# fahmyadan/SMARTS

Hardware: AMD Instinct MI355X
Metric: aggregate env-steps/s (all agents) (higher is better)
Workload: dtype f64; 1 GPU; scenarios/loop, 4096 batched envs x 32 Laner agents, waypoints(4x20, lookahead 32)+neighbours(10, r=50 m) obs, OGM 64x64 @ 50/64 m/px, dt=0.1, auto-reset (BASELINE.json configs[3]); total_envs=4096, envs_per_gpu=4096, vehicles_per_env=32, launch_form=large_one_lane

## Files before the change

### include/smx.h

```cpp
#ifndef SMX_H
#define SMX_H

#include <stdint.h>

#ifdef __cplusplus
extern "C" {
#endif

typedef struct smx_handle_s* smx_handle;

typedef enum smx_status {
  SMX_OK = 0,
  SMX_ERR_INVALID = -1,
  SMX_ERR_HIP = -2,
  SMX_ERR_STATE = -3,
  SMX_ERR_NOMEM = -4
} smx_status;

enum {
  SMX_ACTION_KEEP_LANE = 0,
  SMX_ACTION_SLOW_DOWN = 1,
  SMX_ACTION_CHANGE_LANE_LEFT = 2,
  SMX_ACTION_CHANGE_LANE_RIGHT = 3,
  SMX_ACTION_NONE = -1
// ... 424 lines not shown
                         int32_t max_points, double* out_dev, const smx_outputs* out, void* hip_stream);
int smx_sync(smx_handle h, void* hip_stream);
enum {
  SMX_PHASE_CONTROL = 0,
  SMX_PHASE_SCAN,
  SMX_PHASE_OGM,
  SMX_PHASE_SENSORS,
  SMX_PHASE_COMMIT,
  SMX_PHASE_RESET,
  SMX_PHASE_COUNT
};
int smx_set_timing(smx_handle h, int level);
int smx_read_phase_ms(smx_handle h, float* ms, int32_t max_steps, int32_t* n);
int smx_read_step_ms(smx_handle h, float* ms, int32_t max, int32_t* n);
int smx_last_step_ms(smx_handle h, float* ms);
const char* smx_last_error(smx_handle h);
uint64_t smx_struct_size(int which);
int smx_set_controller_gains(smx_handle h, double heading_gain, double lateral_gain);
enum { SMX_LAUNCH_AUTO = 0, SMX_LAUNCH_SMALL = 1, SMX_LAUNCH_LARGE = 2,
       SMX_LAUNCH_LARGE_ONE_LANE = 3, SMX_LAUNCH_LARGE_TEAMS = 4  };
int smx_set_launch_strategy(smx_handle h, int strategy);
enum { SMX_FORM_SMALL = 0, SMX_FORM_LARGE_TEAMS = 1, SMX_FORM_LARGE_ONE_LANE = 2 };
int smx_launch_form(smx_handle h);
const char* smx_version(void);
void smx_destroy(smx_handle h);

#ifdef __cplusplus
}
#endif
#endif
```

### smarts_amd/_native.py

```python
from __future__ import annotations

import ctypes as C
import os
from typing import Optional

from .build import LIB_PATH

ACTION_KEEP_LANE, ACTION_SLOW_DOWN, ACTION_CHANGE_LANE_LEFT, ACTION_CHANGE_LANE_RIGHT = 0, 1, 2, 3
ACTION_NONE = -1
DONE_COLLISION, DONE_OFF_ROAD, DONE_OFF_ROUTE = 1, 2, 4
DONE_ON_SHOULDER, DONE_WRONG_WAY, DONE_NOT_MOVING = 8, 16, 32
(EV_COLLISIONS, EV_OFF_ROAD, EV_OFF_ROUTE, EV_ON_SHOULDER, EV_WRONG_WAY, EV_NOT_MOVING, EV_REACHED_GOAL,
 EV_REACHED_MAX_EPISODE_STEPS, EV_AGENTS_ALIVE_DONE, EV_COUNT) = range(10)
EVENT_NAMES = ["collisions", "off_road", "off_route", "on_shoulder", "wrong_way", "not_moving", "reached_goal",
               "reached_max_episode_steps", "agents_alive_done"]
EV = {name.upper(): i for i, name in enumerate(EVENT_NAMES)}
ACTION_SPACES = {"Lane": 0, "Continuous": 1, "ActuatorDynamic": 2, "LaneWithContinuousSpeed": 3, "Trajectory": 4,
                 "TargetPose": 5, "TrajectoryWithTime": 6, "MPC": 7, "Imitation": 8}
TRAJ_COLS = 11
SOCIAL_MODELS = {"constant": 0, "idm": 1}
PHASES = ["control", "scan", "ogm", "sensors", "commit", "reset"]
SENSOR_WAYPOINTS, SENSOR_NEIGHBORS, SENSOR_ACCELEROMETER, SENSOR_OGM, SENSOR_LIDAR, SENSOR_DAGM = 1, 2, 4, 8, 16, 32
SENSOR_ROAD_WAYPOINTS = 64
SENSOR_LANE_TTC = 128
# ... 144 lines not shown

def torch_dtype_code(t) -> int:
    import torch

    return {torch.float64: DT_F64, torch.float32: DT_F32, torch.int32: DT_I32, torch.int16: DT_I16, torch.int8: DT_I8,
            torch.uint8: DT_U8, torch.int64: DT_U64, torch.uint64: DT_U64}[t.dtype]


def bind_buffer(struct, names, name, tensor):
    k = names.index(name)
    setattr(struct, name, tensor.data_ptr() if tensor is not None else None)
    struct.count[k] = int(tensor.numel()) if tensor is not None else 0
    struct.dtype[k] = torch_dtype_code(tensor) if tensor is not None else DT_NONE


EXPORTS = [
    "smx_create", "smx_load_map", "smx_set_vias", "smx_set_missions", "smx_step_continuous", "smx_step_trajectory", "smx_read_phase_ms", "smx_set_lidar_rays", "smx_reset", "smx_step", "smx_sync", "smx_last_step_ms",
    "smx_set_timing", "smx_last_error", "smx_version", "smx_destroy", "smx_set_controller_gains", "smx_struct_size", "smx_read_step_ms",
    "smx_check_buffers", "smx_set_launch_strategy", "smx_launch_form", "smx_step_target_pose", "smx_step_trajectory_with_time",
    "smx_set_mission_goals", "smx_check_mission_goals", "smx_actions_to_world", "smx_set_rgb_output", "smx_check_rgb_output",
    "smx_bind_frame_stack", "smx_check_frame_stack", "smx_set_guard", "smx_check_guard",
    "smx_set_social_history", "smx_check_social_history", "smx_set_social_history_dims", "smx_check_social_history_dims",
    "smx_set_history_agents", "smx_check_history_agents", "smx_step_history_agents",
]
LAUNCH_FORMS = {0: "small", 1: "large_teams", 2: "large_one_lane"}
LAUNCH_STRATEGIES = {"auto": 0, "small": 1, "large": 2, "large_one_lane": 3, "large_teams": 4}
OGM_ENV_MIN_VEHICLES = 8192
LARGE_BATCH_VEHICLES = 16384

_lib: Optional[C.CDLL] = None


class NativeLibraryError(RuntimeError):
    pass


def load_library(path: Optional[str] = None) -> C.CDLL:
    global _lib
    if _lib is not None and path is None:
        return _lib
    path = path or os.environ.get("SMX_LIBRARY") or LIB_PATH
    if not os.path.exists(path):
        raise NativeLibraryError(
            f"{path} not found: build it with `python -m smarts_amd.build` (hipcc --offload-arch=gfx950); "
            "smarts_amd has no CPU fallback"
        )
# ... 68 lines not shown
                                             C.c_char_p, C.c_uint64]
    lib.smx_check_history_agents.restype = C.c_int
    lib.smx_step_history_agents.argtypes = [h, C.POINTER(SmxState), C.POINTER(SmxSpawns), C.POINTER(SmxOutputs), _p]
    lib.smx_step_history_agents.restype = C.c_int
    lib.smx_read_phase_ms.argtypes = [h, C.POINTER(C.c_float), _i32, C.POINTER(_i32)]
    lib.smx_read_phase_ms.restype = C.c_int
    lib.smx_set_timing.argtypes = [h, C.c_int]
    lib.smx_set_timing.restype = C.c_int
    lib.smx_set_controller_gains.argtypes = [h, _f64, _f64]
    lib.smx_set_controller_gains.restype = C.c_int
    lib.smx_last_error.argtypes = [h]
    lib.smx_last_error.restype = C.c_char_p
    lib.smx_version.argtypes = []
    lib.smx_version.restype = C.c_char_p
    lib.smx_destroy.argtypes = [h]
    lib.smx_destroy.restype = None
    lib.smx_check_buffers.argtypes = [C.POINTER(SmxConfig), C.c_int, C.POINTER(SmxState), C.POINTER(SmxSpawns),
                                      C.POINTER(SmxOutputs), C.c_char_p, C.c_uint64]
    lib.smx_check_buffers.restype = C.c_int
    lib.smx_set_launch_strategy.argtypes = [h, C.c_int]
    lib.smx_set_launch_strategy.restype = C.c_int
    lib.smx_launch_form.argtypes = [h]
    lib.smx_launch_form.restype = C.c_int
    lib.smx_struct_size.argtypes = [C.c_int]
    lib.smx_struct_size.restype = C.c_uint64
    for which, mirror in enumerate((SmxConfig, SmxMapTables, SmxState, SmxSpawns, SmxOutputs)):
        if lib.smx_struct_size(which) != C.sizeof(mirror):
            raise NativeLibraryError(
                f"ABI mismatch: {mirror.__name__} is {C.sizeof(mirror)} bytes here, "
                f"{lib.smx_struct_size(which)} in {path} (stale build?)"
            )
    _lib = lib
    return lib


class SmxError(RuntimeError):
    pass


def check(lib, handle, rc: int, what: str):
    if rc != 0:
        msg = lib.smx_last_error(handle)
        raise SmxError(f"{what} failed ({rc}): {msg.decode() if msg else ''}")
```

### smarts_amd/csrc/smx_kernels.hip

```cpp
#include <hip/hip_runtime.h>

#include <algorithm>
#include <cmath>
#include <cstdio>
#include <cstdlib>
#include <cstring>
#include <new>
#include <string>
#include <vector>

#include "smx_guard.h"
#include "smx_history.h"
#include "smx_host.h"
#include "smx_plan.h"
#include "smx_scan.h"
#include "smx_vehicle.h"

#define SMX_COLLISION_LEEWAY 0.05
#define SMX_POSE_SCAN_RADIUS 10.0
#define SMX_WPT_PRELOAD 8
#define SMX_SLOW_BLOCKS 512

struct KernelArgs {
  smx_config cfg;
// ... 21 lines not shown
  int debug_skip;
  int wp_blocks, obs_blocks, lidar_blocks;
  double dagm_reach;
  uint8_t* rgb;
  KnotLists knots;
  const KnotRow* knot_table;
  unsigned long long* knot_served;
  MissionsDev missions;
  const int32_t* alive_list;
  const int32_t* alive_count;
  int alive_segmented;
  int32_t* status;
  double* seeds_carry;
  double* facts_carry;
  int32_t* slow_list;
  int32_t* slow_count;
  uint8_t* seed_pending;
  uint8_t* guard;
  GuardBox guard_box;
  HistoryDev history;
  HistoryDimsDev dims;
  float* ha_action;
  uint8_t* ha_status;
};
enum {
  SMX_DEVICE_BAD_LANE_ACTION = 1,
  SMX_DEVICE_BAD_TRAJECTORY = 2,
  SMX_DEVICE_BAD_TARGET_POSE = 4
};

#define SF(field) a.st.f64[(size_t)(field) * total + gid]

#define SMX_SEG_STRIDE 32
__device__ __forceinline__ size_t seg_position(const size_t seg, const size_t off) {
  return ((off >> 6) << 9) | (seg << 6) | (off & 63);
}

__device__ __forceinline__ size_t launch_vehicle(const KernelArgs& a, size_t i, size_t total) {
  if (a.alive_list == nullptr) return i < total ? i : total;
  const int32_t entry = a.alive_list[i < total ? i : total - 1];
  if (a.alive_segmented) {
    const size_t off = ((i >> 9) << 6) | (i & 63);
    return (i < total && off < (size_t)a.alive_count[SMX_SEG_STRIDE * ((i >> 6) & 7)]) ? (size_t)entry : total;
  }
  return i < (size_t)*a.alive_count ? (size_t)entry : total;
}
// ... 2758 lines not shown
      SF(SMX_S_MCL_Y) = so[1];
      fl |= SMX_F_SOCIAL;
    }
  } else if (__builtin_expect(a.history.follow != nullptr, 0)) {
    fl = history_agent_respawn(a, gid, total, episode);
    if constexpr (GUARD) a.guard[gid] = 0;
  }
  a.st.flags[gid] = fl;
  if (a.knots.key != nullptr)
    for (int p = 0; p < SMX_WP_LANES; ++p) a.knots.key[gid * SMX_WP_LANES + p] = -1;
  a.st.facts_i32[(size_t)SMX_FI_TRIP_HAS_WP * total + gid] = 0;
  a.st.steps[gid] = 1;
}

struct __align__(16) SharedPose {
  double x, y, heading, speed;
  double lane_dist;
  int lane;
  int alive;
  short nl, nlidx;
  int pad;
};

__device__ __forceinline__ void zero_dense_rows(const KernelArgs& a, size_t gid, int t, int nth) {
  const smx_config& c = a.cfg;
  const smx_outputs& o = a.out;
  for (int k = t; k < 3; k += nth) o.ego_pos[gid * 3 + k] = 0.0;
  for (int k = t; k < SMX_EGO_F32_COUNT; k += nth) o.ego_f32[gid * SMX_EGO_F32_COUNT + k] = 0.0f;
  for (int k = t; k < 2; k += nth) o.ego_lane[gid * 2 + k] = -1;
  for (int k = t; k < SMX_EV_COUNT; k += nth) o.events[gid * SMX_EV_COUNT + k] = 0;
  if (t == 0) {
    if (o.collidees) o.collidees[gid] = 0ull;
    o.reward[gid] = 0.0;
    o.dist[gid] = 0.0;
  }
  if (c.sensors & SMX_SENSOR_WAYPOINTS) {
    const int per = c.wp_paths * c.wp_len;
    for (int k = t; k < per * 3; k += nth) o.wp_pos[gid * per * 3 + k] = 0.0;
    for (int k = t; k < per; k += nth) {
      const size_t q = gid * per + k;
      o.wp_heading[q] = 0.0f;
      o.wp_lane_width[q] = 0.0f;
      o.wp_speed_limit[q] = 0.0f;
      o.wp_lane_index[q] = 0;
      o.wp_lane_id[q] = -1;
    }
// ... 10 lines not shown
      o.nb_speed[q] = 0.0f;
      o.nb_lane_index[q] = 0;
      o.nb_lane_id[q] = -1;
      o.nb_slot[q] = -1;
    }
    if (t == 0) o.nb_count[gid] = 0;
  }
  if ((c.sensors & SMX_SENSOR_LANE_TTC) && t == 0) o.lane_ttc_flags[gid] = 0;
  if (c.via_max > 0 && o.via_near) {
    for (int k = t; k < c.via_max; k += nth) o.via_near[gid * (size_t)c.via_max + k] = -1;
    if (t == 0) {
      o.via_near_count[gid] = 0;
      o.via_hit[gid] = 0;
    }
  }
  auto zero_bytes = [&](uint8_t* base, size_t n) {
    uint8_t* p = base + gid * n;
    if (n % 16 == 0 && (reinterpret_cast<uintptr_t>(p) & 15) == 0) {
      for (size_t k = t; k < n / 16; k += nth) reinterpret_cast<int4*>(p)[k] = make_int4(0, 0, 0, 0);
    } else {
      for (size_t k = t; k < n; k += nth) p[k] = 0;
    }
  };
  if ((c.sensors & SMX_SENSOR_OGM) && o.ogm) zero_bytes(o.ogm, (size_t)c.ogm_width * c.ogm_height);
  if ((c.sensors & SMX_SENSOR_DAGM) && o.dagm) zero_bytes(o.dagm, (size_t)c.dagm_width * c.dagm_height);
  if ((c.sensors & SMX_SENSOR_LIDAR) && o.lidar_hit) {
    for (int k = t; k < c.lidar_rays; k += nth) o.lidar_hit[gid * (size_t)c.lidar_rays + k] = 0;
    for (int k = t; k < c.lidar_rays * 3; k += nth) o.lidar_point[gid * (size_t)c.lidar_rays * 3 + k] = 0.0;
  }
}

#define SMX_NB_STAGE 16
static_assert(SMX_BLOCK * SMX_NB_STAGE * 3 < 4096, "small_quotient's range");
struct ObsStage {
  float ego_f32[SMX_BLOCK][SMX_EGO_F32_COUNT];
  short ego_lane[SMX_BLOCK][2];
  unsigned char events[SMX_BLOCK][SMX_EV_COUNT + 1];
  signed char nb_list[SMX_BLOCK][SMX_NB_STAGE];
  unsigned char nb_kept[SMX_BLOCK];
  unsigned char mode[SMX_BLOCK];
};

__device__ inline bool drove_off_map(const MissionsDev& ms, const MapDev& m, int n_slots, int lane, double dist, double px,
                                     double py, double heading) {
  if (lane < 0) return false;
  const double offset = lane_offset_along(m, lane, px, py);
  const double width = m.lane_width[lane];
// ... 640 lines not shown
  const double res = c.ogm_resolution;
  const double ex0 = SF(SMX_S_X), ey0 = SF(SMX_S_Y), eh = wrap_heading(SF(SMX_S_HEADING));
  const double rx = cos(eh), ry = sin(eh);
  const double fx = -sin(eh), fy = cos(eh);
  __shared__ OgmMate mates[SMX_BLOCK];
  for (int base = 0; base < n_veh; base += SMX_BLOCK) {
    const int j = base + (int)threadIdx.x;
    bool in_view = false;
    if (j < n_veh) {
      const size_t og = (size_t)env * n_veh + j;
      if (a.st.flags[og] & SMX_F_ALIVE) in_view = ogm_mate_footprint(a, og, total, W, H, res, ex0, ey0, rx, ry, fx, fy, mates[threadIdx.x]);
    }
    unsigned long long todo = __ballot(in_view);
    __syncthreads();
    while (todo != 0ull) {
      const int idx = __ffsll((long long)todo) - 1;
      const OgmMate q = mates[idx];
      todo &= todo - 1ull;
      ogm_draw_mate<255>(a, (size_t)env * n_veh + base + idx, tile, q, W, H, res);
    }
    __syncthreads();
  }
  __syncthreads();
  int4* dst = reinterpret_cast<int4*>(a.out.ogm + gid * (size_t)bytes);
  for (int k = threadIdx.x; k < bytes / 16; k += SMX_BLOCK) dst[k] = reinterpret_cast<const int4*>(tile)[k];
}

struct OgmPose {
  double x, y, ch, sh;
  int alive, observes;
};
#ifndef SMX_SIDE_PRIO
#define SMX_SIDE_PRIO 0
#endif
#define SMX_WAVE_SYNC()                                   \
  do {                                                    \
    __builtin_amdgcn_fence(__ATOMIC_RELEASE, "wavefront"); \
    __builtin_amdgcn_wave_barrier();                      \
    __builtin_amdgcn_fence(__ATOMIC_ACQUIRE, "wavefront"); \
  } while (0)
__device__ __forceinline__ double readlane_f64(double v, int src) {
  const long long b = __double_as_longlong(v);
  const int lo = __builtin_amdgcn_readlane((int)(b & 0xffffffffll), src);
  const int hi = __builtin_amdgcn_readlane((int)(b >> 32), src);
  return __longlong_as_double(((long long)hi << 32) | (unsigned int)lo);
}

template <int OBS, bool SIZED>
// ... 22 lines not shown
    p.sh = sin(h);
    pose[threadIdx.x] = p;
  }
  if (wave == 0) {
    const bool obs_here = lane < n_veh && pose[lane].observes;
    const unsigned long long om = __ballot(obs_here);
    if (obs_here) observers[__popcll(om & ((1ull << lane) - 1ull))] = (unsigned char)lane;
    if (lane == 0) n_observers = __popcll(om);
  }
  __syncthreads();
  unsigned char* tile = tiles + (size_t)wave * OBS * bytes;
  const double res = c.ogm_resolution;
  const double inv_res = 1.0 / res;
  const int half = lane >> 5, in_half = lane & 31;
  const int mate = OBS == 2 ? in_half : lane;
  const int mate_clamped = min(mate, n_veh - 1);
  const VehBox mate_box = vehicle_box(a, (size_t)env * n_veh + mate_clamped, SIZED);
  const double hl = 0.5 * mate_box.length, hw = 0.5 * mate_box.width;
  const int lr = in_half >> 2, lc = in_half & 3;
  const double col_bias = 0.5 - 0.5 * W, row_bias = 0.5 * H - 0.5;
  const int n_obs = n_observers;
  const int per_round = SMX_OGM_WAVES * OBS;
  const int rounds = (n_obs + per_round - 1) / per_round;
#pragma nounroll
  for (int it = 0; it < rounds; ++it) {
    const int turn0 = (it * SMX_OGM_WAVES + wave) * OBS;
    const int n_live = min(OBS, n_obs - turn0);
    if (n_live <= 0) break;
    for (int k = lane; k < n_live * (bytes / 16); k += 64) reinterpret_cast<int4*>(tile)[k] = make_int4(0, 0, 0, 0);
    const int my_turn = turn0 + (OBS == 2 ? half : 0);
    const bool live = my_turn < n_obs;
    const int obs = (int)observers[live ? my_turn : turn0];
    const OgmPose e = pose[obs];
    const OgmPose v = pose[mate_clamped];
    const double rx = e.ch, ry = e.sh;
    const double fx = -e.sh, fy = e.ch;
    const double dx = v.x - e.x, dy = v.y - e.y;
    const double cx = dx * rx + dy * ry, cy = dx * fx + dy * fy;
    const double cm = v.ch, sm = v.sh;
    const double vfx = cm * ry - sm * rx, vfy = sm * ry + cm * rx, vrx = cm * rx + sm * ry, vry = sm * rx - cm * ry;
    const double ext_x = fabs(vfx) * hl + fabs(vrx) * hw, ext_y = fabs(vfy) * hl + fabs(vry) * hw;
    const double slack = 1e-6;
    const double c_lo = fmax((cx - ext_x) * inv_res + 0.5 * W - 0.5 - slack, -1.0), c_hi = fmin((cx + ext_x) * inv_res + 0.5 * W - 0.5 + slack, (double)W);
    const double r_lo = fmax(0.5 * H - 0.5 - (cy + ext_y) * inv_res - slack, -1.0), r_hi = fmin(0.5 * H - 0.5 - (cy - ext_y) * inv_res + slack, (double)H);
    const int c0 = max((int)ceil(c_lo), 0), c1 = min((int)floor(c_hi), W - 1);
    const int r0 = max((int)ceil(r_lo), 0), r1 = min((int)floor(r_hi), H - 1);
// ... 13 lines not shown
      const double qvfx = __shfl(vfx, src), qvfy = __shfl(vfy, src), qvrx = __shfl(vrx, src), qvry = __shfl(vry, src);
      const int qc0 = __shfl(c0, src), qr0 = __shfl(r0, src), qbw = __shfl(bw, src), qbh = __shfl(bh, src);
      double qhl = 0.5 * SMX_CHASSIS_LENGTH, qhw = 0.5 * SMX_CHASSIS_WIDTH;
      if constexpr (SIZED) qhl = __shfl(hl, src), qhw = __shfl(hw, src);
      unsigned char* dst_tile = tile + (OBS == 2 ? (src >> 5) * bytes : 0);
      const int bh_max = max(__builtin_amdgcn_readlane(bh, s0), __builtin_amdgcn_readlane(bh, s1));
      const int bw_max = max(__builtin_amdgcn_readlane(bw, s0), __builtin_amdgcn_readlane(bw, s1));
#pragma clang loop unroll(disable) vectorize(disable) interleave(disable)
      for (int rr = 0; rr < bh_max; rr += 8) {
#pragma clang loop unroll(disable) vectorize(disable) interleave(disable)
        for (int cc = 0; cc < bw_max; cc += 4) {
          const int dr = rr + lr, dc = cc + lc;
          const int r = qr0 + dr, col = qc0 + dc;
          const double py = (row_bias - (double)r) * res - qcy;
          const double px = ((double)col + col_bias) * res - qcx;
          if (drawing && dr < qbh && dc < qbw && fabs(px * qvfx + py * qvfy) <= qhl && fabs(px * qvrx + py * qvry) <= qhw)
            dst_tile[r * W + col] = 255;
        }
      }
    }
    SMX_WAVE_SYNC();
    for (int t = 0; t < n_live; ++t) {
      const int4* src_tile = reinterpret_cast<const int4*>(tile + (size_t)t * bytes);
      int4* dst = reinterpret_cast<int4*>(a.out.ogm + ((size_t)env * n_veh + (int)observers[turn0 + t]) * (size_t)bytes);
      for (int k = lane; k < bytes / 16; k += 64) dst[k] = src_tile[k];
    }
    SMX_WAVE_SYNC();
  }
  SMX_TSTAMP(span1);
  SMX_TSPAN(6, span0, span1);
}

template <int VALUE>
__device__ __forceinline__ void road_layer(const KernelArgs& a, unsigned char* tile, const int W, const int H, const double res,
                                           const double ex0, const double ey0, const double rx, const double ry, const double fx,
                                           const double fy) {
  const MapDev& m = a.map;
  const double vw = 0.5 * W * res, vh = 0.5 * H * res;
  const double reach = sqrt(vw * vw + vh * vh) + a.dagm_reach + 1e-6;
  int cx0 = (int)floor((ex0 - reach - m.sg_x0) / m.sg_cell), cx1 = (int)floor((ex0 + reach - m.sg_x0) / m.sg_cell);
  int cy0 = (int)floor((ey0 - reach - m.sg_y0) / m.sg_cell), cy1 = (int)floor((ey0 + reach - m.sg_y0) / m.sg_cell);
  cx0 = max(cx0, 0);
  cy0 = max(cy0, 0);
  cx1 = min(cx1, m.sg_nx - 1);
  cy1 = min(cy1, m.sg_ny - 1);
  const int wave = threadIdx.x >> 6, lane = threadIdx.x & 63, n_waves = SMX_BLOCK >> 6;
  for (int gy = cy0; gy <= cy1; ++gy) {
    if (cx0 > cx1) break;
// ... 1130 lines not shown
  void* goals_blob;
  std::vector<int32_t> host_route_last;
  MissionsDev missions;
  double heading_gain_pos = 0.04, lateral_gain_pos = 3.4;
  double nb_d2_max;
  int slow_blocks = SMX_SLOW_BLOCKS;
  bool list_ready;
  int seg_parity;
  smx_state list_state;
  int group_parity;
  bool map_junctions;
  double dagm_reach;
  uint8_t* guard_out;
  uint64_t guard_count;
  double guard_margin = SMX_GUARD_MARGIN_DEFAULT;
  GuardBox guard_box = {1.0, 1.0, 0.0, 0.0};
  uint8_t* rgb_out;
  uint64_t rgb_count;
  void* history_blob;
  HistoryDev history;
  float* ha_action;
  uint8_t* ha_status;
  int32_t history_max_id;
  void* dims_blob;
  HistoryDimsDev dims;
  struct StackBinding {
    int32_t source, layout;
    uint8_t* dst;
    uint64_t bytes;
    uint32_t row;
  };
  std::vector<StackBinding> stacks;
  int debug_skip;
  int launch_strategy = SMX_LAUNCH_AUTO;
  bool timing;
  std::vector<hipEvent_t> ev_pool;
  size_t ev_used;
  bool phase_timing;
  std::vector<hipEvent_t> ph_pool;
  size_t ph_used;
  std::string err;
};

static thread_local std::string g_create_err;

static void drop_social_dims(smx_handle h) {
// ... 71 lines not shown
  l.flat = total;
  l.seg = (total + 2 + SMX_SEG_STRIDE - 1) / SMX_SEG_STRIDE * SMX_SEG_STRIDE;
  l.group_count = l.seg + 2 * 8 * SMX_SEG_STRIDE;
  l.groups = l.group_count + 2 * SMX_SEG_STRIDE;
  l.size = l.groups + (size_t)c.num_envs;
  return l;
}

static_assert(SMX_HOST_BLOCK == SMX_BLOCK && SMX_HOST_WP_LANES == SMX_WP_LANES && SMX_HOST_MAX_KNOTS == SMX_MAX_KNOTS &&
                  SMX_HOST_SLOW_BLOCKS == SMX_SLOW_BLOCKS && SMX_HOST_STACK_BLOCK == SMX_STACK_BLOCK,
              "smx_host.h mirrors these");

extern "C" int smx_create(const smx_config* cfg, int device, smx_handle* out) {
  if (out) *out = nullptr;
  if (!cfg || !out) return refuse(g_create_err, "smx_create: null config or handle pointer");
  if (const char* why = config_error(*cfg)) return refuse(g_create_err, why);
  const hipError_t e = hipSetDevice(device);
  if (e != hipSuccess) return refuse(g_create_err, std::string("hipSetDevice: ") + hipGetErrorString(e), SMX_ERR_HIP);
  smx_handle h = new (std::nothrow) smx_handle_s();
  if (!h) return refuse(g_create_err, "out of memory", SMX_ERR_NOMEM);
  h->cfg = *cfg;
  h->device = device;
  h->nb_d2_max = radius_threshold(h->cfg.nb_radius);
#ifdef SMX_DEBUG_TIMING
  if (const char* dbg = getenv("SMX_DEBUG_SKIP")) h->debug_skip = atoi(dbg);
#endif
  *out = h;
  return SMX_OK;
}

extern "C" int smx_set_launch_strategy(smx_handle h, int strategy) {
  if (!h) return SMX_ERR_INVALID;
  if (strategy < SMX_LAUNCH_AUTO || strategy > SMX_LAUNCH_LARGE_TEAMS) return fail(h, SMX_ERR_INVALID, "unknown launch strategy");
  h->launch_strategy = strategy;
  return SMX_OK;
}

static PlanInputs plan_inputs(const smx_handle_s* h, bool is_step, const smx_state* st, bool follow = false) {
  PlanInputs in{};
  in.cfg = &h->cfg;
  in.launch_strategy = h->launch_strategy;
  in.map_junctions = h->map_junctions;
  in.slow_blocks = h->slow_blocks;
  in.routed = h->missions.route_last != nullptr;
  in.is_step = is_step;
  in.phase_timing = h->phase_timing && h->ph_used < 16384;
  in.side_ready = h->side_ready;
  in.list_carried = st && h->list_ready && std::memcmp(&h->list_state, st, sizeof(smx_state)) == 0;
  in.debug_skip = (SMX_SKIP(*h, SMX_SKIP_FORCE_SMALL) ? SMX_SKIP_FORCE_SMALL : 0) |
                  (SMX_SKIP(*h, SMX_SKIP_FORCE_SCAN_SPLIT) ? SMX_SKIP_FORCE_SCAN_SPLIT : 0);
  in.alive_blob = h->alive_blob != nullptr;
  in.knots_blob = h->knots_blob != nullptr;
  in.knot_table = h->knot_table != nullptr && h->knot_table_mode != 0;
  in.ctrl_blob = h->ctrl_blob != nullptr;
  in.pending_blob = h->pending_blob;
  in.slow = SlowLists{h->slow_blob, (size_t)h->cfg.num_envs * h->cfg.num_vehicles};
  in.slow_parity = h->alive_parity;
  in.frame_stack_bound = !h->stacks.empty();
  in.guard_bound = h->guard_out != nullptr;
  in.dims_bound = h->dims.table != nullptr;
  in.history_bound = h->history.vehicle != nullptr;
  in.follow_entry = follow;
  return in;
}

extern "C" int smx_launch_form(smx_handle h) {
  if (!h) return SMX_ERR_INVALID;
  if (!h->map_loaded) return fail(h, SMX_ERR_STATE, "smx_launch_form needs the map (the form depends on it)");
  return tick_plan(plan_inputs(h, false, nullptr)).form;
}

extern "C" int smx_set_controller_gains(smx_handle h, double heading_gain, double lateral_gain) {
  if (!h) return SMX_ERR_INVALID;
  h->heading_gain_pos = heading_gain;
  h->lateral_gain_pos = lateral_gain;
  return SMX_OK;
}

extern "C" int smx_load_map(smx_handle h, const smx_map_tables* t) {
  if (!h || !t) return SMX_ERR_INVALID;
  if (const char* why = map_tables_error(*t)) return fail(h, SMX_ERR_INVALID, why);
  if (h->guard_out && !guard_map_ok(*t, h->guard_margin))
    return fail(h, SMX_ERR_INVALID, "state guard: with this margin a cell index of this map's grids would not fit (smx_guard.h, SMX_GUARD_INDEX_MAX)");
  SMX_HIP(hipSetDevice(h->device));
  h->dagm_reach = map_dagm_reach(*t);
// ... 767 lines not shown
  a.wp_pool_limit = h->wp_pool_limit;
  a.lateral_gain_pos = h->lateral_gain_pos;
  a.debug_skip = h->debug_skip;
  a.knots = h->knots;
  a.knot_table = p.knot_table ? h->knot_table : nullptr;
  a.knot_served = (p.knot_table && h->knot_table_mode == 2) ? (unsigned long long*)(h->knot_stats + 2) : nullptr;
  a.status = h->status_dev;
  a.alive_list = nullptr;
  a.alive_count = nullptr;
  a.alive_segmented = 0;
  a.slow_list = nullptr;
  a.slow_count = nullptr;
  a.seed_pending = nullptr;
  a.seeds_carry = h->scan_carry;
  a.facts_carry = h->scan_carry ? h->scan_carry + 4 * total : nullptr;
  a.dagm_reach = h->dagm_reach;
  a.rgb = h->rgb_out;
  a.guard = h->guard_out;
  a.guard_box = h->guard_box;
  a.history = h->history;
  a.dims = h->dims;
  a.ha_action = h->ha_action;
  a.ha_status = h->ha_status;
  a.wp_blocks = (int)p.wp_blocks;
  a.obs_blocks = (int)p.obs_blocks;
  a.lidar_blocks = (int)p.lidar_blocks;
  return a;
}

enum class Entry { RESET, LANE, FLOATS, TRAJECTORY, TARGET_POSE, TRAJECTORY_WITH_TIME, HISTORY_AGENTS };
static int enqueue(smx_handle h, const Entry entry, const int8_t* actions, const float* actions_f32, const double* traj,
                   const int32_t* traj_n, int32_t traj_max, const uint8_t* mask, const smx_state* st,
                   const smx_spawns* sp, const smx_outputs* out, void* stream_) {
  if (!h) return SMX_ERR_INVALID;
  if (!h->map_loaded) return fail(h, SMX_ERR_STATE, "smx_load_map has not been called");
  int rc = check_buffers(h, st, sp, out);
  if (rc != SMX_OK) return rc;
  const bool is_step = entry != Entry::RESET;
  const bool follow = entry == Entry::HISTORY_AGENTS;
  if (follow) {
    if (h->history.follow == nullptr) return fail(h, SMX_ERR_STATE, "smx_step_history_agents: no history agents are bound (smx_set_history_agents)");
  } else if (is_step) {
    const int sp_ = h->cfg.action_space;
    const bool ok = sp_ == SMX_ACTION_SPACE_LANE ? (entry == Entry::LANE && actions != nullptr)
                    : (sp_ == SMX_ACTION_SPACE_TRAJECTORY || sp_ == SMX_ACTION_SPACE_MPC)
                        ? (entry == Entry::TRAJECTORY && traj != nullptr && traj_n != nullptr)
// ... 12 lines not shown
  KernelArgs a = kernel_args(h, p, actions, actions_f32, traj, traj_n, traj_max, mask, st, sp, out);
  const bool timed = h->timing && is_step && h->ev_used < 65536;
  if (timed) {
    if (h->ev_pool.size() < 2 * (h->ev_used + 1)) {
      hipEvent_t e0, e1;
      SMX_HIP(hipEventCreate(&e0));
      SMX_HIP(hipEventCreate(&e1));
      h->ev_pool.push_back(e0);
      h->ev_pool.push_back(e1);
    }
    SMX_HIP(hipEventRecord(h->ev_pool[2 * h->ev_used], stream));
  }
  hipEvent_t* ph = nullptr;
  if (p.phased) {
    const size_t need = (h->ph_used + 1) * (SMX_PHASE_COUNT + 1);
    while (h->ph_pool.size() < need) {
      hipEvent_t e;
      SMX_HIP(hipEventCreate(&e));
      h->ph_pool.push_back(e);
    }
    ph = &h->ph_pool[h->ph_used * (SMX_PHASE_COUNT + 1)];
    SMX_HIP(hipEventRecord(ph[0], stream));
  }
  if (p.social) launch(k_social, p.veh_blocks, 0, stream, a);
  alive_list(h, p, a, stream);
  if (is_step) {
    launch_control(h, p, a, stream);
    if (ph) SMX_HIP(hipEventRecord(ph[SMX_PHASE_CONTROL + 1], stream));
    observation_pass(h, p, a, stream, ph);
  }
  rc = tail_and_reset_pass(h, p, a, mask, st, stream, ph);
  if (rc != SMX_OK) return rc;
  if (p.frame_stack) {
    rc = launch_frame_stacks(h, is_step, mask, st, out, stream);
    if (rc != SMX_OK) return rc;
  }
  SMX_HIP(hipGetLastError());
  if (ph) {
    SMX_HIP(hipEventRecord(ph[SMX_PHASE_RESET + 1], stream));
    h->ph_used += 1;
  }
  if (timed) {
    SMX_HIP(hipEventRecord(h->ev_pool[2 * h->ev_used + 1], stream));
    h->ev_used += 1;
  }
  return SMX_OK;
// ... 114 lines not shown

extern "C" int smx_debug_set_knot_table(smx_handle h, int32_t mode) {
  if (!h) return SMX_ERR_INVALID;
  if (mode < 0 || mode > 2) return fail(h, SMX_ERR_INVALID, "smx_debug_set_knot_table: 0 (walked lists), 1 (table), 2 (table, counting)");
  h->knot_table_mode = mode;
  return SMX_OK;
}

extern "C" int smx_debug_knot_table_stats(smx_handle h, int64_t* out4) {
  if (!h || !out4) return SMX_ERR_INVALID;
  if (!h->knot_table) return fail(h, SMX_ERR_STATE, "no knot table (no map loaded, or no waypoints sensor)");
  SMX_HIP(hipDeviceSynchronize());
  int32_t st[4];
  SMX_HIP(hipMemcpy(st, h->knot_stats, sizeof(st), hipMemcpyDeviceToHost));
  unsigned long long served;
  std::memcpy(&served, st + 2, sizeof(served));
  out4[0] = h->map.n_lanepoints;
  out4[1] = st[0];
  out4[2] = st[1];
  out4[3] = (int64_t)served;
  return SMX_OK;
}

extern "C" int smx_set_timing(smx_handle h, int level) {
  if (!h) return SMX_ERR_INVALID;
  h->timing = level == 1;
  h->phase_timing = level == 2;
  return SMX_OK;
}

extern "C" int smx_read_phase_ms(smx_handle h, float* ms, int32_t max_steps, int32_t* n) {
  if (!h || !ms || !n || max_steps < 0) return SMX_ERR_INVALID;
  int32_t count = 0;
  for (size_t i = 0; i < h->ph_used; ++i) {
    hipEvent_t* ph = &h->ph_pool[i * (SMX_PHASE_COUNT + 1)];
    SMX_HIP(hipEventSynchronize(ph[SMX_PHASE_COUNT]));
    if (count >= max_steps) continue;
    for (int p = 0; p < SMX_PHASE_COUNT; ++p) {
      float t = 0.f;
      SMX_HIP(hipEventElapsedTime(&t, ph[p], ph[p + 1]));
      ms[(size_t)count * SMX_PHASE_COUNT + p] = t;
    }
    ++count;
  }
  h->ph_used = 0;
  *n = count;
// ... 33 lines not shown
  if (h->scan_carry) (void)hipFree(h->scan_carry);
  if (h->slow_blob) (void)hipFree(h->slow_blob);
  if (h->pending_blob) (void)hipFree(h->pending_blob);
  if (h->spill_blob) (void)hipFree(h->spill_blob);
  if (h->knot_table) (void)hipFree(h->knot_table);
  if (h->knot_stats) (void)hipFree(h->knot_stats);
  if (h->ctrl_blob) (void)hipFree(h->ctrl_blob);
  if (h->status_dev) (void)hipFree(h->status_dev);
  if (h->side_ready) {
    for (int i = 0; i < 3; ++i) {
      (void)hipStreamSynchronize(h->side[i]);
      (void)hipStreamDestroy(h->side[i]);
      (void)hipEventDestroy(h->ev_join[i]);
    }
    (void)hipEventDestroy(h->ev_fork);
    (void)hipEventDestroy(h->ev_fork_grid);
  }
  if (h->vias_dev) (void)hipFree(h->vias_dev);
  if (h->via_off_dev) (void)hipFree(h->via_off_dev);
  if (h->missions_blob) (void)hipFree(h->missions_blob);
  if (h->goals_blob) (void)hipFree(h->goals_blob);
  if (h->history_blob) (void)hipFree(h->history_blob);
  if (h->dims_blob) (void)hipFree(h->dims_blob);
  for (hipEvent_t e : h->ev_pool) (void)hipEventDestroy(e);
  for (hipEvent_t e : h->ph_pool) (void)hipEventDestroy(e);
  delete h;
}
```

### smarts_amd/csrc/smx_plan.h

```cpp
#pragma once
#include <stddef.h>
#include <stdint.h>

#include "../../include/smx.h"

#define SMX_BLOCK 64
#define SMX_WP_LANES 4
#ifndef SMX_TEAM
#define SMX_TEAM 8
#endif
#ifndef SMX_TEAM_LARGE
#define SMX_TEAM_LARGE 4
#endif
#define SMX_WPT_MAX_PATHS 8
#define SMX_OGM_WAVES 4
#define SMX_TTC_TEAM 16
#define SMX_EC_TEAM 16
#define SMX_LARGE_BATCH_VEHICLES 16384
#ifndef SMX_SCAN_WIDE_MAX_VEHICLES
#define SMX_SCAN_WIDE_MAX_VEHICLES 65536
#endif
#ifndef SMX_ONE_LANE_ON_SPLIT_MAPS
#define SMX_ONE_LANE_ON_SPLIT_MAPS 0
#endif
#ifndef SMX_ONE_LANE_MIN_VEHICLES
#define SMX_ONE_LANE_MIN_VEHICLES 114688
#endif
#ifndef SMX_OGM_ENV_MIN_VEHICLES
#define SMX_OGM_ENV_MIN_VEHICLES 8192
#endif
#ifndef SMX_FACTS_EARLY_MAX
#define SMX_FACTS_EARLY_MAX 32768
#endif
#define SMX_SKIP_FORCE_SMALL 131072
#define SMX_SKIP_FORCE_SCAN_SPLIT 65536

struct SlowLists {
  enum { FACTS, SEEDS, CONTROL, ROWS, COUNT };
// ... 10 lines not shown
};

struct PlanInputs {
  const smx_config* cfg;
  int launch_strategy;
  bool map_junctions;
  int slow_blocks;
  bool routed;
  bool is_step;
  bool phase_timing;
  bool side_ready;
  bool list_carried;
  int debug_skip;
  bool alive_blob, knots_blob, ctrl_blob;
  bool knot_table;
  uint8_t* pending_blob;
  SlowLists slow;
  int slow_parity;
  bool frame_stack_bound;
  bool guard_bound;
  bool history_bound;
  bool dims_bound;
  bool follow_entry;
};

enum class AliveList : uint8_t { NONE, CARRIED, BUILD };
enum class Control : uint8_t { NONE, ONE, ONE_LDS, PATHS_LAW, LAW, FAST_LISTED, KINEMATIC, KINEMATIC_FOLLOW };
static constexpr bool smx_kinematic_space(int action_space) {
  constexpr unsigned kinematic = (1u << SMX_ACTION_SPACE_TARGET_POSE) | (1u << SMX_ACTION_SPACE_TRAJECTORY_WITH_TIME) |
                                 (1u << SMX_ACTION_SPACE_IMITATION);
  return ((kinematic >> (action_space & 31)) & 1u) != 0;
}
enum class Seeds : uint8_t { SCAN, ONE_LANE, ROUTED, WIDE, FOUR };
enum class Facts : uint8_t { SCAN, ONE_LANE, WIDE, FOUR };
enum class FactsStart : uint8_t { CALLER, WITH_GRIDS, AFTER_SEEDS };
enum class Rows : uint8_t { SENSORS, UNSTAGED, TABLES, EMIT, EMIT_CHAIN_SIDE, EMIT_CHAIN_AFTER };
enum class SlowChain : uint8_t { NONE, SIDE, AFTER_ROWS };
enum class Ogm : uint8_t { NONE, IN_SENSORS, ENV2, ENV1, PER_OBSERVER };
enum class Lidar : uint8_t { NONE, IN_SENSORS, SIDE, CALLER };

struct TickPlan {
  int form;
  bool is_step, phased, routed;
  bool social;
  AliveList alive;
  int32_t* alive_zero;
  Control control;
  SlowRef control_slow;
  bool fork;
  bool scan_split;
  Seeds team_seeds;
  Facts facts;
  FactsStart facts_start;
  Rows rows;
  bool chain_fused;
  SlowRef facts_slow, seeds_slow, rows_slow;
  Ogm ogm;
  Lidar lidar;
  bool dagm, road_waypoints;
  bool rgb;
  size_t rgb_lds;
  bool lane_ttc;
  unsigned ttc_blocks, ttc_first_blocks;
  size_t ttc_lds;
  bool ego_centric;
  unsigned ec_blocks, ec_first_blocks;
  bool frame_stack;
  bool guard;
  bool sized;
  bool tail_builds_list;
  bool tail_grids;
  bool reset_pass, lidar_first, first_walks_new;
  bool knot_table;
  unsigned veh_blocks, wp_blocks, obs_blocks, env_blocks, lidar_blocks, seeds_blocks, facts_blocks, slow_blocks, sensor_blocks;
  size_t ogm_bytes, dagm_bytes, ogm_lds, sensor_lds;
  uint8_t* pending;

  bool small() const { return form == SMX_FORM_SMALL; }
  SlowChain chain() const {
    return rows == Rows::EMIT_CHAIN_SIDE ? SlowChain::SIDE : rows == Rows::EMIT_CHAIN_AFTER ? SlowChain::AFTER_ROWS : SlowChain::NONE;
// ... 54 lines not shown
  p.facts_start = !p.fork ? FactsStart::CALLER : total <= SMX_FACTS_EARLY_MAX ? FactsStart::WITH_GRIDS : FactsStart::AFTER_SEEDS;
  const bool one_lane_seeds = one_lane && !in.routed && staged && in.pending_blob &&
                              (in.launch_strategy == SMX_LAUNCH_LARGE_ONE_LANE || total >= SMX_ONE_LANE_MIN_VEHICLES);
  p.rows = small ? Rows::SENSORS
           : !staged ? Rows::UNSTAGED
           : !one_lane ? Rows::TABLES
           : !one_lane_seeds ? Rows::EMIT
           : p.fork ? Rows::EMIT_CHAIN_SIDE : Rows::EMIT_CHAIN_AFTER;
  p.chain_fused = p.rows == Rows::EMIT_CHAIN_SIDE && !in.map_junctions;
  p.pending = in.pending_blob;

  p.ogm_bytes = (c.sensors & SMX_SENSOR_OGM) ? (size_t)c.ogm_width * c.ogm_height : 0;
  p.dagm_bytes = (c.sensors & SMX_SENSOR_DAGM) ? (size_t)c.dagm_width * c.dagm_height : 0;
  const bool env2_fits = c.num_vehicles <= 32 && p.ogm_bytes * SMX_OGM_WAVES * 2 <= 64 * 1024;
  if (!p.ogm_bytes)
    p.ogm = Ogm::NONE;
  else if (env2_fits && (!small || total >= SMX_OGM_ENV_MIN_VEHICLES))
    p.ogm = Ogm::ENV2;
  else if (small)
    p.ogm = p.ogm_bytes <= 16 * 1024 ? Ogm::IN_SENSORS : Ogm::PER_OBSERVER;
  else
    p.ogm = p.ogm_bytes * SMX_OGM_WAVES <= 64 * 1024 ? Ogm::ENV1 : Ogm::PER_OBSERVER;
  p.ogm_lds = p.ogm == Ogm::ENV2 ? p.ogm_bytes * SMX_OGM_WAVES * 2 : p.ogm == Ogm::ENV1 ? p.ogm_bytes * SMX_OGM_WAVES : p.ogm_bytes;
  p.dagm = p.dagm_bytes != 0;
  p.rgb = (c.sensors & SMX_SENSOR_RGB) != 0;
  p.rgb_lds = p.rgb ? (size_t)c.rgb_width * c.rgb_height : 0;
  p.lidar = !lidar ? Lidar::NONE : small ? Lidar::IN_SENSORS : p.fork ? Lidar::SIDE : Lidar::CALLER;
  p.road_waypoints = (c.sensors & SMX_SENSOR_ROAD_WAYPOINTS) != 0;
  p.lane_ttc = (c.sensors & SMX_SENSOR_LANE_TTC) != 0;

  p.tail_builds_list = !small && in.alive_blob && in.slow.base && !idm && !in.history_bound;
  p.reset_pass = !in.is_step || c.auto_reset;
  p.tail_grids = p.reset_pass && (p.ogm_bytes || p.dagm_bytes || p.rgb);
  p.lidar_first = p.reset_pass && lidar && !small;
  const bool table = in.knot_table && !in.routed && staged && c.wp_lookahead >= 16;
  p.knot_table = table && one_lane;
  p.first_walks_new = p.reset_pass && !small && one_lane_cut && staged && !(table && p.form == SMX_FORM_LARGE_ONE_LANE);

  const int vpb = SMX_BLOCK / SMX_WP_LANES, epb = SMX_BLOCK / c.num_vehicles;
  p.veh_blocks = smx_blocks(total);
  p.wp_blocks = smx_blocks(total, vpb);
  p.obs_blocks = (unsigned)((c.num_envs + epb - 1) / epb);
  p.env_blocks = smx_blocks((size_t)c.num_envs);
  p.lidar_blocks = lidar ? (unsigned)total : 0;
  p.slow_blocks = (unsigned)in.slow_blocks;
  p.seeds_blocks = small ? (p.scan_split ? 2 : 1) * smx_blocks(total * SMX_TEAM)
// ... 23 lines not shown
```

### smarts_amd/engine.py

```python
from __future__ import annotations

import ctypes as C
import math
from dataclasses import dataclass, field
from typing import Dict, Optional, Sequence, Tuple

import numpy as np
import torch

from . import _native as nat
from .lidar import SensorParams, base_rays, ray_count
from .map_compiler import CompiledMap


def checked_guard_margin(margin):
    m = margin
    if isinstance(m, bool) or not isinstance(m, (int, float)) or not math.isfinite(m) or not 0.0 <= m <= nat.GUARD_MARGIN_MAX:
        raise ValueError(f"state_guard_margin must be a finite number of metres in [0, {nat.GUARD_MARGIN_MAX:g}], got {m!r}")
    return m


@dataclass
class SimConfig:

# ... 475 lines not shown
            if nat.GOAL_TRAVERSE in kinds:
                from .missions import lane_end_tables

                h, d = lane_end_tables(self.cm)
                n_lanes = len(h)
                heading = np.ascontiguousarray(h, dtype=np.float64).ctypes.data_as(C.POINTER(C.c_double))
                dead_end = np.ascontiguousarray(d, dtype=np.int32).ctypes.data_as(C.POINTER(C.c_int32))
                keep = (h, d)
            nat.check(self.lib, self.handle, self.lib.smx_set_mission_goals(self.handle, goals, N, heading, dead_end, n_lanes),
                      "smx_set_mission_goals")

    def bind_rgb(self, images: Optional[torch.Tensor]):
        if images is None:
            nat.check(self.lib, self.handle, self.lib.smx_set_rgb_output(self.handle, None, 0), "smx_set_rgb_output")
            self.out.pop("rgb", None)
            return
        want = (self.E, self.N, self.cfg.rgb_height, self.cfg.rgb_width, 3)
        if images.dtype != torch.uint8 or not images.is_cuda or not images.is_contiguous() or tuple(images.shape) != want:
            raise ValueError(f"the rgb buffer must be a contiguous uint8 device tensor of shape {want}")
        rc = self.lib.smx_set_rgb_output(self.handle, images.data_ptr(), int(images.numel()))
        nat.check(self.lib, self.handle, rc, "smx_set_rgb_output")
        self.out["rgb"] = images

    def bind_guard(self, guard: Optional[torch.Tensor], margin: Optional[float] = None):
        if guard is None:
            nat.check(self.lib, self.handle, self.lib.smx_set_guard(self.handle, None, 0, 0.0), "smx_set_guard")
            self.out.pop("guard", None)
            return
        if guard.dtype != torch.uint8 or tuple(guard.shape) != (self.E, self.N) or guard.device != self.device or not guard.is_contiguous():
            raise ValueError(f"the guard buffer must be a contiguous uint8 device tensor of shape {(self.E, self.N)}")
        margin = float(self.cfg.state_guard_margin if margin is None else margin)
        rc = self.lib.smx_set_guard(self.handle, guard.data_ptr(), int(guard.numel()), margin)
        nat.check(self.lib, self.handle, rc, "smx_set_guard")
        self.out["guard"] = guard

    def set_traffic_history(self, table, start_frames: Optional[torch.Tensor] = None, replaced: Optional[torch.Tensor] = None,
                            dims: bool = False):
        if table is None:
            nat.check(self.lib, self.handle, self.lib.smx_set_social_history(self.handle, None), "smx_set_social_history")
            self.traffic_history = self.history_start_frames = self.history_replaced = None
            self.history_dims = False
            self._drop_history_agents()
            return
        E = self.E
        if start_frames is None:
            start_frames = torch.zeros((1, E), dtype=torch.int32, device=self.device)
# ... 292 lines not shown
```

Before: 11.13 million env-steps/s.

## Write only changed non-zero OGM pieces using a persistent per-tile occupancy mask

Adds a device bitmask per OGM tile that records which 64-byte pieces were non-zero on the previous step. When storing a tile, a piece is written only if it is non-zero now or was non-zero before, so mostly-empty grids skip global stores of zeros. The mask is reset to all-ones whenever the output buffer changes or the caller invalidates it, and it is zeroed on env reset. The trade-off is that the output buffer is assumed not to be modified externally between steps, and each store now does an extra ballot and mask read/write.

```diff
diff --git a/include/smx.h b/include/smx.h
--- a/include/smx.h
+++ b/include/smx.h
@@ -470,6 +470,8 @@
 int smx_set_launch_strategy(smx_handle h, int strategy);
 enum { SMX_FORM_SMALL = 0, SMX_FORM_LARGE_TEAMS = 1, SMX_FORM_LARGE_ONE_LANE = 2 };
 int smx_launch_form(smx_handle h);
+int smx_invalidate_outputs(smx_handle h);
+int smx_set_ogm_delta(smx_handle h, int on);
 const char* smx_version(void);
 void smx_destroy(smx_handle h);
 
diff --git a/smarts_amd/_native.py b/smarts_amd/_native.py
--- a/smarts_amd/_native.py
+++ b/smarts_amd/_native.py
@@ -190,6 +190,7 @@
     "smx_bind_frame_stack", "smx_check_frame_stack", "smx_set_guard", "smx_check_guard",
     "smx_set_social_history", "smx_check_social_history", "smx_set_social_history_dims", "smx_check_social_history_dims",
     "smx_set_history_agents", "smx_check_history_agents", "smx_step_history_agents",
+    "smx_invalidate_outputs", "smx_set_ogm_delta",
 ]
 LAUNCH_FORMS = {0: "small", 1: "large_teams", 2: "large_one_lane"}
 LAUNCH_STRATEGIES = {"auto": 0, "small": 1, "large": 2, "large_one_lane": 3, "large_teams": 4}
@@ -304,6 +305,10 @@
     lib.smx_set_launch_strategy.restype = C.c_int
     lib.smx_launch_form.argtypes = [h]
     lib.smx_launch_form.restype = C.c_int
+    lib.smx_invalidate_outputs.argtypes = [h]
+    lib.smx_invalidate_outputs.restype = C.c_int
+    lib.smx_set_ogm_delta.argtypes = [h, C.c_int]
+    lib.smx_set_ogm_delta.restype = C.c_int
     lib.smx_struct_size.argtypes = [C.c_int]
     lib.smx_struct_size.restype = C.c_uint64
     for which, mirror in enumerate((SmxConfig, SmxMapTables, SmxState, SmxSpawns, SmxOutputs)):
diff --git a/smarts_amd/csrc/smx_kernels.hip b/smarts_amd/csrc/smx_kernels.hip
--- a/smarts_amd/csrc/smx_kernels.hip
+++ b/smarts_amd/csrc/smx_kernels.hip
@@ -67,6 +67,7 @@
   HistoryDimsDev dims;
   float* ha_action;
   uint8_t* ha_status;
+  unsigned long long* ogm_mask;
 };
 enum {
   SMX_DEVICE_BAD_LANE_ACTION = 1,
@@ -2871,6 +2872,53 @@
   int pad;
 };
 
+#define SMX_OGM_LPP (SMX_OGM_PIECE / 16)
+#define SMX_OGM_PPS (64 / SMX_OGM_LPP)
+__device__ __forceinline__ unsigned long long ogm_pieces_of_lanes(unsigned long long b) {
+  if constexpr (SMX_OGM_LPP == 1) return b;
+  b |= b >> 1;
+  b |= b >> 2;
+  b &= 0x1111111111111111ull;
+  b = (b | (b >> 3)) & 0x0303030303030303ull;
+  b = (b | (b >> 6)) & 0x000f000f000f000full;
+  b = (b | (b >> 12)) & 0x000000ff000000ffull;
+  return (b | (b >> 24)) & 0xffffull;
+}
+__device__ __forceinline__ unsigned long long ogm_lanes_of_pieces(unsigned long long q) {
+  if constexpr (SMX_OGM_LPP == 1) return q;
+  q &= 0xffffull;
+  q = (q | (q << 24)) & 0x000000ff000000ffull;
+  q = (q | (q << 12)) & 0x000f000f000f000full;
+  q = (q | (q << 6)) & 0x0303030303030303ull;
+  q = (q | (q << 3)) & 0x1111111111111111ull;
+  return q * 0xfull;
+}
+__device__ __forceinline__ void ogm_store_tile(const int4* src, int4* dst, unsigned long long* mask, const int n16, const int lane) {
+  if (mask == nullptr) {
+    for (int k = lane; k < n16; k += 64) dst[k] = src[k];
+    return;
+  }
+  const int steps = (n16 + 63) >> 6;
+  unsigned long long old_word = 0ull, new_word = 0ull;
+#pragma nounroll
+  for (int i = 0; i < steps; ++i) {
+    const int k = i * 64 + lane;
+    const bool mine = k < n16;
+    int4 v = make_int4(0, 0, 0, 0);
+    if (mine) v = src[k];
+    const unsigned long long nz = ogm_pieces_of_lanes(__ballot((v.x | v.y | v.z | v.w) != 0));
+    const int sub = i % SMX_OGM_LPP, shift = sub * SMX_OGM_PPS;
+    if (sub == 0) {
+      old_word = mask[i / SMX_OGM_LPP];
+      new_word = 0ull;
+    }
+    const unsigned long long leaving = ogm_lanes_of_pieces(nz | (old_word >> shift));
+    if (mine && ((leaving >> lane) & 1ull)) dst[k] = v;
+    new_word |= nz << shift;
+    if ((sub == SMX_OGM_LPP - 1 || i == steps - 1) && lane == 0) mask[i / SMX_OGM_LPP] = new_word;
+  }
+}
+
 __device__ __forceinline__ void zero_dense_rows(const KernelArgs& a, size_t gid, int t, int nth) {
   const smx_config& c = a.cfg;
   const smx_outputs& o = a.out;
@@ -2927,7 +2975,13 @@
       for (size_t k = t; k < n; k += nth) p[k] = 0;
     }
   };
-  if ((c.sensors & SMX_SENSOR_OGM) && o.ogm) zero_bytes(o.ogm, (size_t)c.ogm_width * c.ogm_height);
+  if ((c.sensors & SMX_SENSOR_OGM) && o.ogm) {
+    zero_bytes(o.ogm, (size_t)c.ogm_width * c.ogm_height);
+    if (a.ogm_mask) {
+      const size_t words = smx_ogm_mask_words((size_t)c.ogm_width * c.ogm_height);
+      for (size_t k = t; k < words; k += nth) a.ogm_mask[gid * words + k] = 0ull;
+    }
+  }
   if ((c.sensors & SMX_SENSOR_DAGM) && o.dagm) zero_bytes(o.dagm, (size_t)c.dagm_width * c.dagm_height);
   if ((c.sensors & SMX_SENSOR_LIDAR) && o.lidar_hit) {
     for (int k = t; k < c.lidar_rays; k += nth) o.lidar_hit[gid * (size_t)c.lidar_rays + k] = 0;
@@ -3614,8 +3668,10 @@
     __syncthreads();
   }
   __syncthreads();
+  static_assert(SMX_BLOCK == 64, "ogm_store_tile: the workgroup is one wavefront");
   int4* dst = reinterpret_cast<int4*>(a.out.ogm + gid * (size_t)bytes);
-  for (int k = threadIdx.x; k < bytes / 16; k += SMX_BLOCK) dst[k] = reinterpret_cast<const int4*>(tile)[k];
+  ogm_store_tile(reinterpret_cast<const int4*>(tile), dst, a.ogm_mask ? a.ogm_mask + gid * smx_ogm_mask_words((size_t)bytes) : nullptr,
+                 bytes / 16, (int)threadIdx.x);
 }
 
 struct OgmPose {
@@ -3684,6 +3740,7 @@
   const int n_obs = n_observers;
   const int per_round = SMX_OGM_WAVES * OBS;
   const int rounds = (n_obs + per_round - 1) / per_round;
+  const size_t mask_words = smx_ogm_mask_words((size_t)bytes);
 #pragma nounroll
   for (int it = 0; it < rounds; ++it) {
     const int turn0 = (it * SMX_OGM_WAVES + wave) * OBS;
@@ -3743,8 +3800,9 @@
     SMX_WAVE_SYNC();
     for (int t = 0; t < n_live; ++t) {
       const int4* src_tile = reinterpret_cast<const int4*>(tile + (size_t)t * bytes);
-      int4* dst = reinterpret_cast<int4*>(a.out.ogm + ((size_t)env * n_veh + (int)observers[turn0 + t]) * (size_t)bytes);
-      for (int k = lane; k < bytes / 16; k += 64) dst[k] = src_tile[k];
+      const size_t gid = (size_t)env * n_veh + (int)observers[turn0 + t];
+      int4* dst = reinterpret_cast<int4*>(a.out.ogm + gid * (size_t)bytes);
+      ogm_store_tile(src_tile, dst, a.ogm_mask ? a.ogm_mask + gid * mask_words : nullptr, bytes / 16, lane);
     }
     SMX_WAVE_SYNC();
   }
@@ -4921,6 +4979,11 @@
   float* ha_action;
   uint8_t* ha_status;
   int32_t history_max_id;
+  unsigned long long* ogm_mask;
+  size_t ogm_mask_bytes;
+  const uint8_t* ogm_rows;
+  bool ogm_known;
+  bool ogm_delta = true;
   void* dims_blob;
   HistoryDimsDev dims;
   struct StackBinding {
@@ -5038,6 +5101,15 @@
   h->cfg = *cfg;
   h->device = device;
   h->nb_d2_max = radius_threshold(h->cfg.nb_radius);
+  if (h->cfg.sensors & SMX_SENSOR_OGM) {
+    h->ogm_mask_bytes = (size_t)cfg->num_envs * cfg->num_vehicles * smx_ogm_mask_words((size_t)cfg->ogm_width * cfg->ogm_height) * sizeof(unsigned long long);
+    const hipError_t em = hipMalloc((void**)&h->ogm_mask, h->ogm_mask_bytes);
+    if (em != hipSuccess) {
+      h->ogm_mask = nullptr;
+      smx_destroy(h);
+      return refuse(g_create_err, std::string("hipMalloc (OGM piece mask): ") + hipGetErrorString(em), SMX_ERR_HIP);
+    }
+  }
 #ifdef SMX_DEBUG_TIMING
   if (const char* dbg = getenv("SMX_DEBUG_SKIP")) h->debug_skip = atoi(dbg);
 #endif
@@ -5077,6 +5149,7 @@
   in.dims_bound = h->dims.table != nullptr;
   in.history_bound = h->history.vehicle != nullptr;
   in.follow_entry = follow;
+  in.ogm_mask = h->ogm_mask != nullptr && h->ogm_delta;
   return in;
 }
 
@@ -5890,6 +5963,7 @@
   a.dims = h->dims;
   a.ha_action = h->ha_action;
   a.ha_status = h->ha_status;
+  a.ogm_mask = (p.ogm_delta && out->ogm) ? h->ogm_mask : nullptr;
   a.wp_blocks = (int)p.wp_blocks;
   a.obs_blocks = (int)p.obs_blocks;
   a.lidar_blocks = (int)p.lidar_blocks;
@@ -5948,6 +6022,12 @@
     ph = &h->ph_pool[h->ph_used * (SMX_PHASE_COUNT + 1)];
     SMX_HIP(hipEventRecord(ph[0], stream));
   }
+  if (a.ogm_mask && !(h->ogm_known && h->ogm_rows == out->ogm)) {
+    SMX_HIP(hipMemsetAsync(h->ogm_mask, 0xff, h->ogm_mask_bytes, stream));
+    h->ogm_rows = out->ogm;
+    h->ogm_known = true;
+  }
+  if (!a.ogm_mask) h->ogm_known = false;
   if (p.social) launch(k_social, p.veh_blocks, 0, stream, a);
   alive_list(h, p, a, stream);
   if (is_step) {
@@ -6108,6 +6188,19 @@
   return SMX_OK;
 }
 
+extern "C" int smx_invalidate_outputs(smx_handle h) {
+  if (!h) return SMX_ERR_INVALID;
+  h->ogm_known = false;
+  return SMX_OK;
+}
+
+extern "C" int smx_set_ogm_delta(smx_handle h, int on) {
+  if (!h) return SMX_ERR_INVALID;
+  h->ogm_delta = on != 0;
+  h->ogm_known = false;
+  return SMX_OK;
+}
+
 extern "C" int smx_set_timing(smx_handle h, int level) {
   if (!h) return SMX_ERR_INVALID;
   h->timing = level == 1;
@@ -6187,6 +6280,7 @@
   if (h->goals_blob) (void)hipFree(h->goals_blob);
   if (h->history_blob) (void)hipFree(h->history_blob);
   if (h->dims_blob) (void)hipFree(h->dims_blob);
+  if (h->ogm_mask) (void)hipFree(h->ogm_mask);
   for (hipEvent_t e : h->ev_pool) (void)hipEventDestroy(e);
   for (hipEvent_t e : h->ph_pool) (void)hipEventDestroy(e);
   delete h;
diff --git a/smarts_amd/csrc/smx_plan.h b/smarts_amd/csrc/smx_plan.h
--- a/smarts_amd/csrc/smx_plan.h
+++ b/smarts_amd/csrc/smx_plan.h
@@ -14,6 +14,11 @@
 #endif
 #define SMX_WPT_MAX_PATHS 8
 #define SMX_OGM_WAVES 4
+#ifndef SMX_OGM_PIECE
+#define SMX_OGM_PIECE 64
+#endif
+static_assert(SMX_OGM_PIECE == 16 || SMX_OGM_PIECE == 64, "a piece is one int4 or one 64-byte sector");
+static constexpr size_t smx_ogm_mask_words(size_t tile_bytes) { return (tile_bytes / SMX_OGM_PIECE + 63) / 64; }
 #define SMX_TTC_TEAM 16
 #define SMX_EC_TEAM 16
 #define SMX_LARGE_BATCH_VEHICLES 16384
@@ -70,6 +75,7 @@
   bool history_bound;
   bool dims_bound;
   bool follow_entry;
+  bool ogm_mask;
 };
 
 enum class AliveList : uint8_t { NONE, CARRIED, BUILD };
@@ -104,6 +110,7 @@
   bool chain_fused;
   SlowRef facts_slow, seeds_slow, rows_slow;
   Ogm ogm;
+  bool ogm_delta;
   Lidar lidar;
   bool dagm, road_waypoints;
   bool rgb;
@@ -204,6 +211,7 @@
   else
     p.ogm = p.ogm_bytes * SMX_OGM_WAVES <= 64 * 1024 ? Ogm::ENV1 : Ogm::PER_OBSERVER;
   p.ogm_lds = p.ogm == Ogm::ENV2 ? p.ogm_bytes * SMX_OGM_WAVES * 2 : p.ogm == Ogm::ENV1 ? p.ogm_bytes * SMX_OGM_WAVES : p.ogm_bytes;
+  p.ogm_delta = in.ogm_mask && p.ogm_bytes != 0 && p.ogm_bytes % SMX_OGM_PIECE == 0;
   p.dagm = p.dagm_bytes != 0;
   p.rgb = (c.sensors & SMX_SENSOR_RGB) != 0;
   p.rgb_lds = p.rgb ? (size_t)c.rgb_width * c.rgb_height : 0;
diff --git a/smarts_amd/engine.py b/smarts_amd/engine.py
--- a/smarts_amd/engine.py
+++ b/smarts_amd/engine.py
@@ -521,6 +521,19 @@
         nat.check(self.lib, self.handle, rc, "smx_set_rgb_output")
         self.out["rgb"] = images
 
+    def invalidate_outputs(self):
+        nat.check(self.lib, self.handle, self.lib.smx_invalidate_outputs(self.handle), "smx_invalidate_outputs")
+
+    def set_ogm_delta(self, on: bool):
+        nat.check(self.lib, self.handle, self.lib.smx_set_ogm_delta(self.handle, 1 if on else 0), "smx_set_ogm_delta")
+
+    def bind_ogm(self, tiles: torch.Tensor):
+        want = (self.E, self.N, self.cfg.ogm_height, self.cfg.ogm_width)
+        if not self.cfg.ogm or tiles.dtype != torch.uint8 or tiles.device != self.device or not tiles.is_contiguous() or tuple(tiles.shape) != want:
+            raise ValueError(f"the OGM rows must be a contiguous uint8 device tensor of shape {want} (SimConfig(ogm=True))")
+        nat.bind_buffer(self._out, nat.OUTPUT_BUFFERS, "ogm", tiles)
+        self.out["ogm"] = tiles
+
     def bind_guard(self, guard: Optional[torch.Tensor], margin: Optional[float] = None):
         if guard is None:
             nat.check(self.lib, self.handle, self.lib.smx_set_guard(self.handle, None, 0, 0.0), "smx_set_guard")
```

Result: faster. 11.63 million env-steps/s (median of 6 runs) (+4.4%).
